# trustbloc/fabric-mod

Measured on AMD Instinct MI355X. Metric: ECDSA P-256 verifies/sec (whole node), higher is better.
Workload: dtype int64; 1 GPU; BASELINE.json configs[1]: block of 10000 tx x 3 endorsements = 30000 P-256 tuples per GPU, verify-only kernel via the C ABI, fresh keypair per signatu; tuples_per_gpu=30000, tx_per_block=10000, endorsements_per_tx=3, seed=20260921, parallelism=1 block per GPU, clock_warmup_launches=100

## Files before the change

fabric-mod_amd/csrc/fabgpu_api.hip:

```cpp
#include <hip/hip_runtime.h>
#include <stdlib.h>
#include <string.h>

#include <algorithm>
#include <atomic>
#include <chrono>
#include <condition_variable>
#include <initializer_list>
#include <memory>
#include <sys/mman.h>
#include <set>
#include <mutex>
#include <new>
#include <map>
#include <string>
#include <thread>
#include <vector>

#include "../../include/fabgpu.h"
#include "kernels.h"
#include "key_slots.h"
#include "keyed_fence.h"
#include "block_walk_dev.h"
#include "described_plan.h"
// ... 119 lines not shown
using HipKeyedFence = KeyedFence<HipFenceDev>;

}

struct fabgpu_ctx {
    int device = 0;
    bool allow_pair = true;
    bool allow_quad = true;
    bool nym_side_stream = true;
    std::atomic<bool> test_nym_side_after{false};
    bool nym_two_phase = true;
    bool allow_wide = true;
    int pair_table_lds = -1;
    bool pair_solo = false;
    bool pair_dbl1 = false;
    hipStream_t stream = nullptr;
    int fault = 0;
    int32_t* d_gtab = nullptr;
    uint32_t* d_gtab384 = nullptr;
    std::mutex gtab384_mu;
    std::mutex mu;
    Buf fields;
    Buf arena;
    Buf offs;
    Buf out;
    hipEvent_t ev0 = nullptr, ev1 = nullptr;
    bool timed = false;
    bool time_kernels = false;
    struct QWs {
        void* p = nullptr;
// ... 261 lines not shown
        default: return "unknown fabgpu error";
    }
}

int fabgpu_device_count(fabgpu_ctx*) {
    int n = 0;
    if (hipGetDeviceCount(&n) != hipSuccess) return FABGPU_ENODEV;
    return n;
}

int fabgpu_init(const fabgpu_cfg* cfg, fabgpu_ctx** out) {
    if (!out) return FABGPU_EINVAL;
    *out = nullptr;
    if (cfg && (cfg->flags & ~(uint32_t)(FABGPU_FLAG_ONE_LANE_ONLY | FABGPU_FLAG_TIME_KERNELS | FABGPU_FLAG_NO_QUAD | FABGPU_FLAG_PAIR_TABLE_LDS |
                                          FABGPU_FLAG_PAIR_TABLE_GLOBAL | FABGPU_FLAG_NO_WIDE | FABGPU_FLAG_NYM_FUSED_HASH | FABGPU_FLAG_NYM_NO_SIDE_STREAM |
                                          FABGPU_FLAG_KEY_TABLES_16BIT | FABGPU_FLAG_PAIR_SOLO | FABGPU_FLAG_PAIR_DBL1 | FABGPU_FLAG_P384_WIDE |
                                          FABGPU_FLAG_P384_KEY_TABLES_16BIT)) != 0) return FABGPU_EINVAL;
    if (cfg && (cfg->flags & FABGPU_FLAG_PAIR_TABLE_LDS) && (cfg->flags & FABGPU_FLAG_PAIR_TABLE_GLOBAL)) return FABGPU_EINVAL;
    int ndev = 0;
    if (hipGetDeviceCount(&ndev) != hipSuccess || ndev <= 0) return FABGPU_ENODEV;
    int dev = cfg ? cfg->device : -1;
    if (dev < 0) {
        if (hipGetDevice(&dev) != hipSuccess) return FABGPU_ENODEV;
    }
    if (dev >= ndev) return FABGPU_EINVAL;
    hipDeviceProp_t prop;
    if (hipGetDeviceProperties(&prop, dev) != hipSuccess) return FABGPU_ENODEV;
    if (strncmp(prop.gcnArchName, "gfx950", 6) != 0) return FABGPU_ENODEV;
    fabgpu_ctx* ctx = new (std::nothrow) fabgpu_ctx();
    if (!ctx) return FABGPU_ENOMEM;
    ctx->device = dev;
    ctx->walk_map.flags = hipHostMallocMapped | hipHostMallocCoherent;
    ctx->allow_pair = !(cfg && (cfg->flags & FABGPU_FLAG_ONE_LANE_ONLY));
    ctx->allow_quad = !(cfg && (cfg->flags & FABGPU_FLAG_NO_QUAD));
    ctx->nym_two_phase = !(cfg && (cfg->flags & FABGPU_FLAG_NYM_FUSED_HASH));
    ctx->nym_side_stream = !(cfg && (cfg->flags & FABGPU_FLAG_NYM_NO_SIDE_STREAM));
    ctx->key_tables_16 = cfg && (cfg->flags & FABGPU_FLAG_KEY_TABLES_16BIT);
    ctx->allow_wide = ctx->allow_pair && !(cfg && (cfg->flags & FABGPU_FLAG_NO_WIDE));
    ctx->pair_table_lds = cfg && (cfg->flags & FABGPU_FLAG_PAIR_TABLE_LDS) ? 1 : (cfg && (cfg->flags & FABGPU_FLAG_PAIR_TABLE_GLOBAL) ? 0 : pair_table_default());
    ctx->pair_solo = cfg && (cfg->flags & FABGPU_FLAG_PAIR_SOLO);
    ctx->pair_dbl1 = cfg && (cfg->flags & FABGPU_FLAG_PAIR_DBL1);
    if (std::max<size_t>(prop.sharedMemPerBlock, prop.maxSharedMemoryPerMultiProcessor) < (ctx->pair_solo ? pair_table_lds_solo_bytes() : pair_table_lds_bytes()))
        ctx->pair_table_lds = 0;
    ctx->time_kernels = cfg && (cfg->flags & FABGPU_FLAG_TIME_KERNELS);
    DeviceGuard g(dev);
    int rc = FABGPU_OK;
    do {
        if (hipStreamCreateWithFlags(&ctx->stream, hipStreamNonBlocking) != hipSuccess) { rc = FABGPU_ENODEV; break; }
        if (hipStreamCreateWithFlags(&ctx->stream2, hipStreamNonBlocking) != hipSuccess) { rc = FABGPU_ENODEV; break; }
        if (hipEventCreateWithFlags(&ctx->ev_up, hipEventDisableTiming) != hipSuccess) { rc = FABGPU_ENODEV; break; }
        if (hipStreamCreateWithFlags(&ctx->stream3, hipStreamNonBlocking) != hipSuccess) { rc = FABGPU_ENODEV; break; }
        if (hipStreamCreateWithFlags(&ctx->stream4, hipStreamNonBlocking) != hipSuccess) { rc = FABGPU_ENODEV; break; }
        if (hipStreamCreateWithFlags(&ctx->stream_copy, hipStreamNonBlocking) != hipSuccess) { rc = FABGPU_ENODEV; break; }
        {
            bool ok = true;
            for (auto& sc : ctx->stream_copy_more) ok = ok && hipStreamCreateWithFlags(&sc, hipStreamNonBlocking) == hipSuccess;
// ... 165 lines not shown
    if (hipEventElapsedTime(&ms, ctx->ev0, ctx->ev1) != hipSuccess) return -1.0f;
    return ms;
}
extern "C" {

int fabgpu_p256_verify_batch_dev(fabgpu_ctx* ctx, size_t n, const void* qx, const void* qy, const void* e, const void* r,
                                 const void* s, void* verdict_bits, void* status, void* stream) {
    if (!ctx || (n && (!qx || !qy || !e || !r || !s || !verdict_bits))) return FABGPU_EINVAL;
    if (dev_too_big(n)) return FABGPU_ETOOBIG;
    if (n == 0) return FABGPU_OK;
    DeviceGuard g(ctx->device);
    hipStream_t st = (hipStream_t)stream;
    VerifyLaunch v = verify_launch_common(ctx, n, r, s, verdict_bits, status);
    v.qx = qx; v.qy = qy;
    v.e = e;
    v.table_lds = ctx->pair_table_lds; v.pair_solo = ctx->pair_solo; v.pair_dbl1 = ctx->pair_dbl1;
    return timed_launch(ctx, st, verify_workspace_bytes((uint32_t)n, ctx->allow_pair), [&](void* wsp) {
        v.qws = wsp;
        return launch_verify(v, st);
    });
}

int fabgpu_sha256_batch_dev(fabgpu_ctx* ctx, size_t n, const void* arena, size_t arena_bytes, const void* off, void* digests,
                            void* stream) {
    if (!ctx || (n && (!arena || !off || !digests))) return FABGPU_EINVAL;
    if (dev_too_big(n, arena_bytes)) return FABGPU_ETOOBIG;
    if (n == 0) return FABGPU_OK;
    DeviceGuard g(ctx->device);
    hipStream_t st = (hipStream_t)stream;
    return timed_launch(ctx, st, 0, [&](void*) { return launch_sha256_batch((uint32_t)n, arena, arena_bytes, off, digests, st); });
}
// ... 2678 lines not shown
        v.n = tot.creators;
        v.e = dt + T.dig.off; v.r = a.r; v.s = a.s;
        v.gtab = ctx->d_gtab;
        v.verdict_bits = dt + T.bitc.off; v.status = dt + T.dst.off;
        v.allow_pair = true; v.lds_reserve = exclusive ? 84u << 10 : 0u;
        hipError_t e;
        if (keyed) {
            v.key_id = a.key_id; v.nkeys = nkeys; v.ktabs = (const void*)kt;
            e = launch_verify(v, s2);
        } else {
            size_t wi = 0;
            void* wsp = nullptr;
            int r2 = ctx->acquire_qws(verify_workspace_bytes(tot.creators, true), &wi, &wsp, s2);
            if (r2 != FABGPU_OK) return r2;
            v.qx = a.qx; v.qy = a.qy; v.qws = wsp;
            v.table_lds = ctx->pair_table_lds; v.pair_solo = ctx->pair_solo; v.pair_dbl1 = ctx->pair_dbl1;
            e = launch_verify(v, s2);
            ctx->release_qws(wi, s2);
        }
        return hip_to_rc(e);
    };
    auto finish = [&]() -> int {
        if (++ctx->walk_seq == 0) ++ctx->walk_seq;
        ho.seq = ctx->walk_seq;
        if (err == hipSuccess && nym_ran) err = hipStreamWaitEvent(st, ctx->ev_w[6], 0);
        if (err == hipSuccess && memo) err = hipMemsetAsync(dt + T.mslots.off, 0, T.mslots.bytes, st);
        if (err == hipSuccess && memo) err = hipMemsetAsync(&((WalkMemoTotals*)(dt + T.mtot.off))->live, 0, 4, st);
        mark("finish: memsets queued");
        if (!memo && !out.tuples && !out.tuple_digest && !out.tuple_qxy && !(has_nym_rows && out.nym_issuer) && walk_small_finish_fits(a, nc)) {
            if (err == hipSuccess) err = launch_walk_status_finish_small(a, nc, ho, st);
            mark("finish: last kernel queued");
// ... 399 lines not shown
```

fabric-mod_amd/csrc/kernels.h:

```cpp
#pragma once
#include <hip/hip_runtime_api.h>
#include <stddef.h>
#include <stdint.h>

namespace fab {
constexpr int KTAB_STRIDE = 4;
constexpr int KEY_SLOT_BITS = 12;
constexpr uint32_t KTAB_GEN_NONE = 0xFFFFFFFFu;
constexpr int VERIFY_BLOCK = 256;
constexpr int VERIFY_MAX_WGS = 256;
constexpr int VERIFY_PAIR_MAX = 32768;
constexpr size_t QWS_UINT4_PER_LANE = (size_t)16 * 8;
constexpr size_t QWS_PAIR_UINT4_PER_SIG = (size_t)16 * 8;

struct ShaPrefixArgs {
    uint32_t m = 0;
    const void* pre_off = nullptr;
    const void* pre_idx = nullptr;
    void* mid_scratch = nullptr;
    bool spans = false;
    void* digests = nullptr;
    bool mid_ready = false;
    uint32_t lds_reserve = 0;
};
// ... 19 lines not shown
    const void *qx = nullptr, *qy = nullptr;
    void* qws = nullptr;
    const void *key_id = nullptr, *ktabs = nullptr;
    uint32_t nkeys = 0;
    const void* e = nullptr;
    const void *arena = nullptr, *off = nullptr;
    size_t arena_bytes = 0;
    ShaPrefixArgs pa;
    const void *r = nullptr, *s = nullptr, *gtab = nullptr;
    void *verdict_bits = nullptr, *status = nullptr;
    bool allow_pair = false;
    uint32_t lds_reserve = 0;
    int table_lds = 0;
    bool pair_solo = false;
    bool pair_dbl1 = false;
};
hipError_t launch_verify(const VerifyLaunch& v, hipStream_t st);

constexpr int WIDE_LAUNCH_MAX = 8192;
constexpr size_t WIDE_SCRATCH_BYTES = 144;
constexpr uint32_t SPREAD_NONE = 0xFFFFFFFFu;
uint32_t spread_waves_per_cu(uint32_t wavefronts);
hipError_t launch_p256_wide_pre(uint32_t n, const void* key_id, uint32_t nkeys, const void* ktabs, const void* r, const void* s, const void* gtab,
                                void* scratch, hipStream_t st, uint32_t lds_spread = 0);
hipError_t launch_p256_wide_post(uint32_t n, const void* e, const void* r, const void* gtab, const void* scratch, void* verdict_bits, void* status,
                                 hipStream_t st, uint32_t lds_spread = 0);
hipError_t launch_sha256_messages(uint32_t n, const void* arena, size_t arena_bytes, const void* off, const ShaPrefixArgs& pa, hipStream_t st);
constexpr uint32_t SHA_COOP_MAX = 2048;
hipError_t launch_sha256_mixed(uint32_t n, const void* arena, size_t arena_bytes, const void* off, bool pairs, void* digests, hipStream_t st,
                               uint32_t lds_reserve = 0);
// ... 92 lines not shown
```

fabric-mod_amd/csrc/kernels.hip:

```cpp
#include <hip/hip_runtime.h>
#include <stdlib.h>
#include <stdint.h>

#include "device_common.h"
#include "kernels.h"
#include "p256_pair29.h"

namespace fab {


__global__ void __launch_bounds__(256) sha256_midstate_kernel(uint32_t m, const uint32_t* __restrict__ arena32, uint32_t arena_words,
                                                               const uint32_t* __restrict__ pre_off, uint32_t spans, uint32_t* __restrict__ mid) {
    uint32_t p = blockIdx.x * blockDim.x + threadIdx.x;
    bool active = p < m;
    uint32_t pc = active ? p : (m - 1);
    uint32_t start = pre_off[spans ? 2 * pc : pc], len = pre_off[spans ? 2 * pc + 1 : pc + 1] - start;
    uint32_t nfull = active ? (len >> 6) : 0, maxfull = nfull;
#pragma unroll
    for (int o = 32; o >= 1; o >>= 1) {
        uint32_t other = __shfl_xor(maxfull, o, 64);
        maxfull = other > maxfull ? other : maxfull;
    }
    maxfull = __builtin_amdgcn_readfirstlane(maxfull);
    uint32_t h[8];
// ... 60 lines not shown
struct DigestHashed {
    static constexpr bool BEFORE_KEY = true;
    const uint32_t* arena32;
    uint32_t arena_words;
    const uint32_t* off;
    const sha_prefixes pre;
    __device__ __forceinline__ void operator()(u256& ve, const TileRow& t, bool writes) const {
        uint32_t h[8];
        sha256_message(arena32, arena_words, off, pre, t.ic, t.active, h);
        emit_digest(pre, t.i, writes, h);
#pragma unroll
        for (int k = 0; k < 8; k++) ve.w[k] = h[7 - k];
    }
};

template <int LANE_COUNT, class QTab, int W = 5, bool DBL1 = false>
struct FreshKey {
    static constexpr int LANES = LANE_COUNT;
    const uint8_t *qx, *qy;
    const int32_t* gtab;
    QTab qtab;
    struct Row { u256 x, y; };
    __device__ __forceinline__ void load(Row& k, uint32_t ic) const {
        load_be_field(k.x, qx, ic);
        load_be_field(k.y, qy, ic);
    }
    __device__ __forceinline__ uint32_t verify(const Row& k, const u256& e, const u256& r, const u256& s, bool odd) {
        if constexpr (LANES == 1) {
            GTab16 gt{gtab};
            return p256_verify_core29(k.x, k.y, e, r, s, gt, qtab);
        } else {
            return p256_verify_pair29<QTab, W, DBL1>(k.x, k.y, e, r, s, gtab, qtab, odd);
        }
    }
};
template <int LANE_COUNT>
struct RegisteredKey {
    static constexpr int LANES = LANE_COUNT;
    const uint32_t* key_id;
    uint32_t nkeys;
    const int32_t* const* ktabs;
    const int32_t* gtab;
    struct Row { const int32_t *kt, *kt16; bool kok; };
    __device__ __forceinline__ void load(Row& k, uint32_t ic) const {
        const uint32_t kid = key_id[ic], sl = kid & ((1u << KEY_SLOT_BITS) - 1u);
        const bool inr = sl < nkeys;
        const int32_t* const* slot = ktabs + KTAB_STRIDE * (size_t)(inr ? sl : 0);
// ... 43 lines not shown
                                                                    uint8_t* __restrict__ status) {
    using QTab = GlobalQTab29<BLOCK>;
    verify_tiles<BLOCK>(n, DigestGiven{e}, FreshKey<1, QTab>{qx, qy, gtab, QTab::of(qws + (size_t)blockIdx.x * (QWS_UINT4_PER_LANE * BLOCK), threadIdx.x)}, r, s, verdict_bits, status);
}

template <int BLOCK>
__global__ void __launch_bounds__(BLOCK, 1) p256_verify_pair_kernel(uint32_t n, const uint8_t* __restrict__ qx, const uint8_t* __restrict__ qy,
                                                                         const uint8_t* __restrict__ e, const uint8_t* __restrict__ r,
                                                                         const uint8_t* __restrict__ s, const int32_t* __restrict__ gtab,
                                                                         uint4* __restrict__ qws, uint64_t* __restrict__ verdict_bits,
                                                                         uint8_t* __restrict__ status) {
    using QTab = PairQTab<BLOCK / 2>;
    verify_tiles<BLOCK>(n, DigestGiven{e}, FreshKey<2, QTab>{qx, qy, gtab, QTab::of(qws + (size_t)blockIdx.x * (QWS_PAIR_UINT4_PER_SIG * (BLOCK / 2)), threadIdx.x >> 1)}, r, s, verdict_bits, status);
}

template <int BLOCK, bool DBL1 = false>
__global__ void __launch_bounds__(BLOCK, 1) p256_verify_pair_lds_solo_kernel(uint32_t n, const uint8_t* __restrict__ qx, const uint8_t* __restrict__ qy,
                                                                             const uint8_t* __restrict__ e, const uint8_t* __restrict__ r,
                                                                             const uint8_t* __restrict__ s, const int32_t* __restrict__ gtab,
                                                                             uint64_t* __restrict__ verdict_bits, uint8_t* __restrict__ status) {
    extern __shared__ uint4 pair_lds[];
    verify_tiles<BLOCK>(n, DigestGiven{e}, FreshKey<2, PairQTabLds, 4, DBL1>{qx, qy, gtab, PairQTabLds::of(pair_lds, threadIdx.x >> 1)}, r, s, verdict_bits, status);
}

template <int BLOCK, bool DBL1 = false>
__global__ void __launch_bounds__(2 * BLOCK, 1) p256_verify_pair_lds_kernel(uint32_t n, const uint8_t* __restrict__ qx, const uint8_t* __restrict__ qy,
                                                                                 const uint8_t* __restrict__ e, const uint8_t* __restrict__ r,
                                                                                 const uint8_t* __restrict__ s, const int32_t* __restrict__ gtab,
                                                                                 uint64_t* __restrict__ verdict_bits, uint8_t* __restrict__ status) {
    extern __shared__ uint4 pair_lds[];
    using Geom = TileGeom<BLOCK, 2>;
    const bool helper = __builtin_amdgcn_readfirstlane(threadIdx.x) >= (uint32_t)BLOCK;
    const uint32_t lane = threadIdx.x & (uint32_t)(BLOCK - 1);
    const bool odd = Geom::odd(lane);
    const uint32_t sub = Geom::sub(lane);
    PairQTabLds qtab = PairQTabLds::of(pair_lds, sub);
    const PairHandoffLds<BLOCK> hand = PairHandoffLds<BLOCK>::of(reinterpret_cast<uint32_t*>(pair_lds + Geom::PER_WG * PAIR_LDS_CELLS_PER_SIG), lane);
    const uint32_t ntiles = Geom::ntiles(n);
    for (uint32_t tile = blockIdx.x; tile < ntiles; tile += gridDim.x) {
        const TileRow t = Geom::row(tile, sub, n);
        u256 u1;
        uint32_t early = 0;
        pair_pt Qp, T;
        bool q_ok = false, t_inf = true;
        if (helper) {
            u256 ve, vr, vs;
            load_be_field(ve, e, t.ic);
            load_be_field(vr, r, t.ic);
            load_be_field(vs, s, t.ic);
            pair_helper_scalars29(u1, early, ve, vr, vs, hand, odd);
        } else {
            u256 vqx, vqy;
            load_be_field(vqx, qx, t.ic);
            load_be_field(vqy, qy, t.ic);
            q_ok = pair_main_table29(Qp, vqx, vqy, qtab, odd);
        }
        __syncthreads();
        if (helper) {
            pair_helper_comb29(u1, early, gtab, hand, odd);
        } else {
            u256 u2;
            hand.get_u2(u2);
            pair_u2_mult29<PairQTabLds, 4, DBL1>(T, t_inf, u2, Qp, qtab, odd);
        }
        __syncthreads();
        if (!helper) {
            u256 vr;
            load_be_field(vr, r, t.ic);
            uint32_t st = pair_main_finish29(T, t_inf, q_ok, vr, hand, odd);
            Geom::emit(t, n, odd, st, verdict_bits, status);
        }
    }
}

template <int BLOCK>
__global__ void __launch_bounds__(BLOCK, 2) p256_verify_keyed_kernel(uint32_t n, const uint32_t* __restrict__ key_id, uint32_t nkeys,
                                                                          const int32_t* const* __restrict__ ktabs, const uint8_t* __restrict__ e,
                                                                          const uint8_t* __restrict__ r, const uint8_t* __restrict__ s,
// ... 127 lines not shown
    g.block = VERIFY_BLOCK;
    g.pair = allow_pair && n <= (uint32_t)VERIFY_PAIR_MAX;
    uint32_t per_wg = g.pair ? VERIFY_BLOCK / 2 : VERIFY_BLOCK;
    uint32_t tiles = (n + per_wg - 1) / per_wg;
    g.wgs = tiles < (uint32_t)VERIFY_MAX_WGS ? tiles : (uint32_t)VERIFY_MAX_WGS;
    return g;
}
int pair_table_default() { return -1; }
size_t pair_table_lds_bytes() { return (size_t)(VERIFY_BLOCK / 2) * PAIR_LDS_CELLS_PER_SIG * 16 + (size_t)VERIFY_BLOCK * PAIR_HAND_WORDS * 4; }
size_t pair_table_lds_solo_bytes() { return (size_t)(VERIFY_BLOCK / 2) * PAIR_LDS_CELLS_PER_SIG * 16; }
size_t verify_workspace_bytes(uint32_t n, bool allow_pair) {
    VerifyGeom g = verify_geom(n, allow_pair);
    if (g.pair) return (size_t)g.wgs * (g.block / 2) * QWS_PAIR_UINT4_PER_SIG * 16;
    return (size_t)g.wgs * g.block * QWS_UINT4_PER_LANE * 16;
}

hipError_t launch_verify(const VerifyLaunch& v, hipStream_t st) {
    const uint32_t n = v.n;
    if (n == 0) return hipSuccess;
    const bool keyed = v.key_id != nullptr && v.ktabs != nullptr, fresh = v.qx != nullptr && v.qy != nullptr;
    const bool hashed = v.off != nullptr, given = v.e != nullptr;
    if (keyed == fresh || hashed == given || keyed != (v.key_id != nullptr || v.ktabs != nullptr) || fresh != (v.qx != nullptr || v.qy != nullptr) ||
        (hashed && v.arena == nullptr && v.arena_bytes != 0))
        return hipErrorInvalidValue;
    const uint8_t *qx = (const uint8_t*)v.qx, *qy = (const uint8_t*)v.qy, *e = (const uint8_t*)v.e, *r = (const uint8_t*)v.r, *s = (const uint8_t*)v.s;
    const uint32_t *key_id = (const uint32_t*)v.key_id, *arena32 = (const uint32_t*)v.arena, *off = (const uint32_t*)v.off;
    const uint32_t arena_words = (uint32_t)((v.arena_bytes + 3) / 4);
    const int32_t* const* ktabs = (const int32_t* const*)v.ktabs;
    const int32_t* gtab = (const int32_t*)v.gtab;
    uint4* qws = (uint4*)v.qws;
    uint64_t* verdict_bits = (uint64_t*)v.verdict_bits;
    uint8_t* status = (uint8_t*)v.status;
    sha_prefixes pre{};
    if (hashed) pre = launch_midstates(v.arena, v.arena_bytes, v.pa, st);
    VerifyGeom g = verify_geom(n, v.allow_pair);
    dim3 grid(g.wgs), block(g.block);
    const uint32_t lds_reserve = hashed ? v.pa.lds_reserve : v.lds_reserve;
    if (!hashed && !keyed) {
        const bool table_lds = v.table_lds < 0 ? n > (uint32_t)PAIR_TABLE_LDS_FROM : v.table_lds != 0;
        if (g.pair && table_lds && !v.pair_solo && !v.pair_dbl1)
            hipLaunchKernelGGL(p256_verify_pair_lds_kernel<VERIFY_BLOCK>, grid, dim3(2 * VERIFY_BLOCK), pair_table_lds_bytes(), st, n, qx, qy, e, r, s, gtab, verdict_bits, status);
        else if (g.pair && table_lds && !v.pair_solo)
            hipLaunchKernelGGL((p256_verify_pair_lds_kernel<VERIFY_BLOCK, true>), grid, dim3(2 * VERIFY_BLOCK), pair_table_lds_bytes(), st, n, qx, qy, e, r, s, gtab, verdict_bits, status);
        else if (g.pair && table_lds && !v.pair_dbl1)
            hipLaunchKernelGGL(p256_verify_pair_lds_solo_kernel<VERIFY_BLOCK>, grid, block, pair_table_lds_solo_bytes(), st, n, qx, qy, e, r, s, gtab, verdict_bits, status);
        else if (g.pair && table_lds)
            hipLaunchKernelGGL((p256_verify_pair_lds_solo_kernel<VERIFY_BLOCK, true>), grid, block, pair_table_lds_solo_bytes(), st, n, qx, qy, e, r, s, gtab, verdict_bits, status);
        else if (g.pair)
            hipLaunchKernelGGL(p256_verify_pair_kernel<VERIFY_BLOCK>, grid, block, lds_reserve, st, n, qx, qy, e, r, s, gtab, qws, verdict_bits, status);
        else
            hipLaunchKernelGGL(p256_verify_kernel<VERIFY_BLOCK>, grid, block, lds_reserve, st, n, qx, qy, e, r, s, gtab, qws, verdict_bits, status);
        return hipGetLastError();
    }
    if (hashed && !keyed) {
        if (g.pair)
            hipLaunchKernelGGL(sha256_p256_verify_pair_kernel<VERIFY_BLOCK>, grid, block, lds_reserve, st, n, arena32, arena_words, off, qx, qy, r, s, gtab, qws,
                               verdict_bits, status, pre);
        else
            hipLaunchKernelGGL(sha256_p256_verify_kernel<VERIFY_BLOCK>, grid, block, lds_reserve, st, n, arena32, arena_words, off, qx, qy, r, s, gtab, qws,
                               verdict_bits, status, pre);
        return hipGetLastError();
    }
    if (!hashed) {
// ... 6 lines not shown
    if (g.pair)
        hipLaunchKernelGGL(sha256_p256_verify_keyed_pair_kernel<VERIFY_BLOCK>, grid, block, lds_reserve, st, n, arena32, arena_words, off, key_id, v.nkeys, ktabs,
                           r, s, gtab, verdict_bits, status, pre);
    else
        hipLaunchKernelGGL(sha256_p256_verify_keyed_kernel<VERIFY_BLOCK>, grid, block, lds_reserve, st, n, arena32, arena_words, off, key_id, v.nkeys, ktabs,
                           r, s, gtab, verdict_bits, status, pre);
    return hipGetLastError();
}

int warm_kernel_functions_kernels() {
    int ok = 0;
    hipFuncAttributes a;
    const void* fns[] = {(const void*)p256_verify_kernel<VERIFY_BLOCK>, (const void*)p256_verify_pair_kernel<VERIFY_BLOCK>,
                         (const void*)p256_verify_pair_lds_kernel<VERIFY_BLOCK>, (const void*)p256_verify_pair_lds_solo_kernel<VERIFY_BLOCK>,
                         (const void*)p256_verify_pair_lds_kernel<VERIFY_BLOCK, true>, (const void*)p256_verify_pair_lds_solo_kernel<VERIFY_BLOCK, true>,
                         (const void*)p256_verify_keyed_kernel<VERIFY_BLOCK>,
                         (const void*)p256_verify_keyed_pair_kernel<VERIFY_BLOCK>, (const void*)sha256_p256_verify_keyed_kernel<VERIFY_BLOCK>,
                         (const void*)sha256_p256_verify_keyed_pair_kernel<VERIFY_BLOCK>, (const void*)sha256_p256_verify_pair_kernel<VERIFY_BLOCK>,
                         (const void*)sha256_p256_verify_kernel<VERIFY_BLOCK>, (const void*)sha256_midstate_kernel, (const void*)gather_spans_kernel};
    for (const void* f : fns) ok += hipFuncGetAttributes(&a, f) == hipSuccess ? 1 : 0;
    return ok;
}

}
```

fabric-mod_amd/csrc/p256_pair29.h:

```cpp
#pragma once
#include "p256_verify29.h"
#include "pair29_gcn.h"

namespace fab {

struct pair_pt {
    fe A, B;
};

__device__ __forceinline__ int32_t pair_swap_i32(int32_t v) {
    return __builtin_amdgcn_update_dpp(0, v, 0xB1, 0xF, 0xF, false);
}
__device__ __forceinline__ void pair_swap_fe(fe& r, const fe& a) {
#pragma unroll
    for (int i = 0; i < 9; i++) r.v[i] = pair_swap_i32(a.v[i]);
}
__device__ __forceinline__ void pair_sel(pair_pt& r, bool c, const pair_pt& a, const pair_pt& b) {
    fe_sel(r.A, c, a.A, b.A);
    fe_sel(r.B, c, a.B, b.B);
}

#define PAIR_TMPS __attribute__((unused)) fe tU1, tU2, tU3, tU4, tU6, tW, tH, tRR, tP1, tP2, tT0, tT1, tTD
#define PAIR_DBL(P) PAIR29_DBL((P).A, (P).B, tU1, tU2, tU3, tW, tP1, tP2, tT0, tT1, tTD)
#define PAIR_DBL4(P) PAIR29_DBL4((P).A, (P).B, tU1, tU2, tU3, tP1, tT0, tTD, tW)
// ... 344 lines not shown
        bool special = true;
#pragma unroll
        for (int l = 0; l < 8; l++) special = special & (u2.w[l] == NM2.w[l]);
        if (__any(special)) {
            pair_pt two;
            qtab.load_state(2u, two, odd);
            fe ny;
#pragma unroll
            for (int l = 0; l < 9; l++) ny.v[l] = -two.B.v[l];
            fe_sel(two.B, odd, two.B, ny);
            pair_sel(T, special, two, T);
        }
    }
}

template <class QTab, int W = 5, bool DBL1 = false>
__device__ __forceinline__ void pair_combined_mult29(pair_pt& Rr, bool& r_inf, const u256& u1, const u256& u2, const fe& QX, const fe& QY,
                                                     const int32_t* __restrict__ gtab, const QTab& qtab, bool odd) {
    static_assert(W == 4 || W == 5, "signed 4- or 5-bit windows");
    const fe ONE = {FE29_R1};
    pair_pt Qp;
    Qp.A = QX;
    fe_sel(Qp.B, odd, ONE, QY);
    pair_qtab_build29<QTab, W>(Qp, QX, QY, qtab, odd);
    pair_pt T;
    bool t_inf;
    pair_u2_mult29<QTab, W, DBL1>(T, t_inf, u2, Qp, qtab, odd);

    pair_pt S;
    bool s_inf;
    pair_comb_mult29<GTab16>(S, s_inf, u1, gtab, Qp, odd);
    pair_final_add29(Rr, r_inf, S, s_inf, T, t_inf, odd);
}

template <class KTab = KeyTab8>
__device__ __forceinline__ void pair_combined_mult_keyed29(pair_pt& Rr, bool& r_inf, const u256& u1, const u256& u2,
                                                           const int32_t* __restrict__ gtab, const int32_t* __restrict__ ktab, bool odd) {
    const fe ONE = {FE29_R1};
    fe gx, gy;
    GTab16 gt{gtab};
    gt.load(0, 1u, gx, gy);
    pair_pt seed, S, T;
// ... 13 lines not shown
    fe_sqr(zz, Rr.B);
    fe_to_mont(rm, r);
    fe_mul(rhs, rm, zz);
    pair_swap_fe(rhs_e, rhs);
    fe_sub(d, rhs_e, Rr.A);
    bool ok = fe_is_zero(d);
    add256(r2, r, N);
    fe_to_mont(rm, r2);
    fe_mul(rhs, rm, zz);
    pair_swap_fe(rhs_e, rhs);
    fe_sub(d, rhs_e, Rr.A);
    ok = ok | (lt256(r, PMN) & fe_is_zero(d));
    return ok & !r_inf;
}

template <class QTab, int W = 5, bool DBL1 = false>
__device__ __forceinline__ uint32_t p256_verify_pair29(const u256& qx, const u256& qy, const u256& e, const u256& r, const u256& s,
                                                        const int32_t* __restrict__ gtab, const QTab& qtab, bool odd) {
    const u256 P = FAB_P256_P;
    uint32_t early = range_status(r, s);

    bool q_in_field = lt256(qx, P) & lt256(qy, P);
    fe QX, QY;
    fe_to_mont(QX, qx);
    fe_to_mont(QY, qy);
    bool q_ok = q_in_field & on_curve29(QX, QY);
    if (early == ST_VALID && !q_ok) early = ST_OFF_CURVE;

    u256 u1, u2;
    pair_ecdsa_scalars29(u1, u2, e, r, s, odd);

    pair_pt Rr;
    bool r_inf;
    pair_combined_mult29<QTab, W, DBL1>(Rr, r_inf, u1, u2, QX, QY, gtab, qtab, odd);
    bool ok = pair_x_equals_r29(Rr, r_inf, r);
    uint32_t st = ok ? ST_VALID : ST_BAD_MATH;
    return early != ST_VALID ? early : st;
}

__device__ __forceinline__ uint32_t p256_verify_keyed_pair29(const u256& e, const u256& r, const u256& s, const int32_t* __restrict__ gtab,
                                                              const int32_t* __restrict__ ktab, const int32_t* __restrict__ ktab16, bool odd) {
    uint32_t early = range_status(r, s);
    u256 u1, u2;
    pair_ecdsa_scalars29(u1, u2, e, r, s, odd);
    pair_pt Rr;
    bool r_inf;
    if (__all(ktab16 != nullptr)) pair_combined_mult_keyed29<GTab16>(Rr, r_inf, u1, u2, gtab, ktab16, odd);
    else pair_combined_mult_keyed29<KeyTab8>(Rr, r_inf, u1, u2, gtab, ktab, odd);
    bool ok = pair_x_equals_r29(Rr, r_inf, r);
// ... 26 lines not shown
#pragma unroll
        for (int l = 0; l < 9; l++) s[(9 + l) * LANES] = (uint32_t)S.B.v[l];
        s[18 * LANES] = (s_inf ? 1u : 0u) | (early << 1);
    }
    __device__ __forceinline__ void get_s(pair_pt& S, bool& s_inf, uint32_t& early) const {
#pragma unroll
        for (int l = 0; l < 9; l++) S.A.v[l] = (int32_t)s[l * LANES];
#pragma unroll
        for (int l = 0; l < 9; l++) S.B.v[l] = (int32_t)s[(9 + l) * LANES];
        uint32_t f = s[18 * LANES];
        s_inf = (f & 1u) != 0;
        early = f >> 1;
    }
};

template <class Hand>
__device__ __forceinline__ void pair_helper_scalars29(u256& u1, uint32_t& early, const u256& e, const u256& r, const u256& s, const Hand& hand,
                                                      bool odd) {
    early = range_status(r, s);
    u256 u2;
    pair_ecdsa_scalars29(u1, u2, e, r, s, odd);
    hand.put_u2(u2);
}

template <class Hand>
__device__ __forceinline__ void pair_helper_comb29(const u256& u1, uint32_t early, const int32_t* __restrict__ gtab, const Hand& hand, bool odd) {
    const fe ONE = {FE29_R1};
    fe gx, gy;
    GTab16 gt{gtab};
    gt.load(0, 1u, gx, gy);
    pair_pt seed, S;
    seed.A = gx;
    fe_sel(seed.B, odd, ONE, gy);
    bool s_inf;
    pair_comb_mult29<GTab16>(S, s_inf, u1, gtab, seed, odd);
    hand.put_s(S, s_inf, early);
}

template <class QTab>
__device__ __forceinline__ bool pair_main_table29(pair_pt& Qp, const u256& qx, const u256& qy, const QTab& qtab, bool odd) {
    const u256 P = FAB_P256_P;
    const fe ONE = {FE29_R1};
    bool q_in_field = lt256(qx, P) & lt256(qy, P);
    fe QX, QY;
    fe_to_mont(QX, qx);
    fe_to_mont(QY, qy);
    bool q_ok = q_in_field & on_curve29(QX, QY);
    Qp.A = QX;
    fe_sel(Qp.B, odd, ONE, QY);
    pair_qtab_build29<QTab, 4>(Qp, QX, QY, qtab, odd);
    return q_ok;
}

template <class Hand>
__device__ __forceinline__ uint32_t pair_main_finish29(const pair_pt& T, bool t_inf, bool q_ok, const u256& r, const Hand& hand, bool odd) {
    pair_pt S, Rr;
    bool s_inf, r_inf;
    uint32_t early;
    hand.get_s(S, s_inf, early);
    if (early == ST_VALID && !q_ok) early = ST_OFF_CURVE;
    pair_final_add29(Rr, r_inf, S, s_inf, T, t_inf, odd);
    bool ok = pair_x_equals_r29(Rr, r_inf, r);
    uint32_t st = ok ? ST_VALID : ST_BAD_MATH;
    return early != ST_VALID ? early : st;
}
// ... 3 lines not shown
```

fabric-mod_amd/fabgpu/__init__.py:

```python
from __future__ import annotations

import ctypes
import os
from typing import List, Optional, Sequence, Tuple

import numpy as np

_HERE = os.path.dirname(os.path.abspath(__file__))
_LIB_PATH = os.environ.get("FABGPU_LIB_PATH") or os.path.join(os.path.dirname(_HERE), "lib", "libfabgpu.so")

FABGPU_OK = 0
IDB_SPANS = 1
IDB_ARENA_STAGED = 2
IDB_SHA3_256 = 4
FABGPU_EINVAL = -1
FABGPU_EPOISONED = -6
FLAG_ONE_LANE_ONLY = 1
FLAG_TIME_KERNELS = 2
FLAG_NYM_NO_SIDE_STREAM = 128
FLAG_NYM_FUSED_HASH = 64
FLAG_NO_QUAD = 4
FLAG_PAIR_TABLE_LDS = 8
FLAG_PAIR_TABLE_GLOBAL = 16
FLAG_PAIR_SOLO = 1024
FLAG_PAIR_DBL1 = 2048
FLAG_KEY_TABLES_16BIT = 256
FLAG_NO_WIDE = 32
FLAG_P384_KEY_TABLES_16BIT = 8192
FLAG_P384_WIDE = 4096
ST_VALID, ST_BAD_MATH, ST_HIGH_S, ST_RANGE, ST_OFF_CURVE = 0, 1, 2, 3, 4

_u8p = ctypes.POINTER(ctypes.c_uint8)
_u32p = ctypes.POINTER(ctypes.c_uint32)
_u64p = ctypes.POINTER(ctypes.c_uint64)
_vp = ctypes.c_void_p
_sz = ctypes.c_size_t


class FabgpuError(RuntimeError):
    """Infrastructure failure (non-zero FABGPU_E*): the Go provider would fall back to bccsp/sw."""
# ... 1681 lines not shown
```

include/fabgpu.h:

```cpp
#ifndef FABGPU_H
#define FABGPU_H

#include <stddef.h>
#include <stdint.h>

#ifdef __cplusplus
extern "C" {
#endif

#define FABGPU_ABI_VERSION 6

#define FABGPU_OK 0
#define FABGPU_EINVAL (-1)
#define FABGPU_ENODEV (-2)
#define FABGPU_ENOMEM (-3)
#define FABGPU_ELAUNCH (-4)
#define FABGPU_ETOOBIG (-5)
#define FABGPU_EPOISONED (-6)

#define FABGPU_ST_VALID 0
#define FABGPU_ST_BAD_MATH 1
#define FABGPU_ST_HIGH_S 2
#define FABGPU_ST_RANGE 3
#define FABGPU_ST_OFF_CURVE 4

typedef struct fabgpu_ctx fabgpu_ctx;

#define FABGPU_FLAG_ONE_LANE_ONLY 1u
#define FABGPU_FLAG_NO_QUAD 4u
#define FABGPU_FLAG_TIME_KERNELS 2u
#define FABGPU_FLAG_PAIR_TABLE_LDS 8u
#define FABGPU_FLAG_PAIR_TABLE_GLOBAL 16u
#define FABGPU_FLAG_NO_WIDE 32u

#define FABGPU_FLAG_NYM_FUSED_HASH 64u
#define FABGPU_FLAG_NYM_NO_SIDE_STREAM 128u

#define FABGPU_FLAG_PAIR_SOLO 1024u
#define FABGPU_FLAG_PAIR_DBL1 2048u

#define FABGPU_FLAG_KEY_TABLES_16BIT 256u

#define FABGPU_FLAG_P384_WIDE 4096u

#define FABGPU_FLAG_P384_KEY_TABLES_16BIT 8192u
#define FABGPU_P384_MAX_TABLES16 32

typedef struct fabgpu_cfg {
    int32_t device;
    uint32_t max_batch;
    uint32_t max_arena;
    uint32_t flags;
} fabgpu_cfg;

// ... 205 lines not shown
```

Baseline: 56.89 million verifies/s.

## Use odd-only signed 4-bit window recoding for the u2·Q pair multiplication

Replaces the Booth-style signed 4-bit recoding of u2 with an odd-digit recoding. u2 is first folded to an odd scalar via n−u2 when it is even, so every window is a nonzero odd digit. The Q table then holds only odd multiples (1Q..15Q), built by repeated adds of 2Q. The main loop becomes branch-free with no point-at-infinity tracking, and a special fix-up covers the n−2 edge case. The old path stays available behind a new BOOTH4 flag, and kernel dispatch moves to a lookup table.

```diff
diff --git a/fabric-mod_amd/csrc/fabgpu_api.hip b/fabric-mod_amd/csrc/fabgpu_api.hip
--- a/fabric-mod_amd/csrc/fabgpu_api.hip
+++ b/fabric-mod_amd/csrc/fabgpu_api.hip
@@ -157,6 +157,7 @@
     int pair_table_lds = -1;
     bool pair_solo = false;
     bool pair_dbl1 = false;
+    bool pair_booth4 = false;
     hipStream_t stream = nullptr;
     int fault = 0;
     int32_t* d_gtab = nullptr;
@@ -448,7 +449,7 @@
     *out = nullptr;
     if (cfg && (cfg->flags & ~(uint32_t)(FABGPU_FLAG_ONE_LANE_ONLY | FABGPU_FLAG_TIME_KERNELS | FABGPU_FLAG_NO_QUAD | FABGPU_FLAG_PAIR_TABLE_LDS |
                                           FABGPU_FLAG_PAIR_TABLE_GLOBAL | FABGPU_FLAG_NO_WIDE | FABGPU_FLAG_NYM_FUSED_HASH | FABGPU_FLAG_NYM_NO_SIDE_STREAM |
-                                          FABGPU_FLAG_KEY_TABLES_16BIT | FABGPU_FLAG_PAIR_SOLO | FABGPU_FLAG_PAIR_DBL1 | FABGPU_FLAG_P384_WIDE |
+                                          FABGPU_FLAG_KEY_TABLES_16BIT | FABGPU_FLAG_PAIR_SOLO | FABGPU_FLAG_PAIR_DBL1 | FABGPU_FLAG_PAIR_BOOTH4 | FABGPU_FLAG_P384_WIDE |
                                           FABGPU_FLAG_P384_KEY_TABLES_16BIT)) != 0) return FABGPU_EINVAL;
     if (cfg && (cfg->flags & FABGPU_FLAG_PAIR_TABLE_LDS) && (cfg->flags & FABGPU_FLAG_PAIR_TABLE_GLOBAL)) return FABGPU_EINVAL;
     int ndev = 0;
@@ -474,6 +475,7 @@
     ctx->pair_table_lds = cfg && (cfg->flags & FABGPU_FLAG_PAIR_TABLE_LDS) ? 1 : (cfg && (cfg->flags & FABGPU_FLAG_PAIR_TABLE_GLOBAL) ? 0 : pair_table_default());
     ctx->pair_solo = cfg && (cfg->flags & FABGPU_FLAG_PAIR_SOLO);
     ctx->pair_dbl1 = cfg && (cfg->flags & FABGPU_FLAG_PAIR_DBL1);
+    ctx->pair_booth4 = cfg && (cfg->flags & FABGPU_FLAG_PAIR_BOOTH4);
     if (std::max<size_t>(prop.sharedMemPerBlock, prop.maxSharedMemoryPerMultiProcessor) < (ctx->pair_solo ? pair_table_lds_solo_bytes() : pair_table_lds_bytes()))
         ctx->pair_table_lds = 0;
     ctx->time_kernels = cfg && (cfg->flags & FABGPU_FLAG_TIME_KERNELS);
@@ -669,7 +671,7 @@
     VerifyLaunch v = verify_launch_common(ctx, n, r, s, verdict_bits, status);
     v.qx = qx; v.qy = qy;
     v.e = e;
-    v.table_lds = ctx->pair_table_lds; v.pair_solo = ctx->pair_solo; v.pair_dbl1 = ctx->pair_dbl1;
+    v.table_lds = ctx->pair_table_lds; v.pair_solo = ctx->pair_solo; v.pair_dbl1 = ctx->pair_dbl1; v.pair_booth4 = ctx->pair_booth4;
     return timed_launch(ctx, st, verify_workspace_bytes((uint32_t)n, ctx->allow_pair), [&](void* wsp) {
         v.qws = wsp;
         return launch_verify(v, st);
@@ -3378,7 +3380,7 @@
             int r2 = ctx->acquire_qws(verify_workspace_bytes(tot.creators, true), &wi, &wsp, s2);
             if (r2 != FABGPU_OK) return r2;
             v.qx = a.qx; v.qy = a.qy; v.qws = wsp;
-            v.table_lds = ctx->pair_table_lds; v.pair_solo = ctx->pair_solo; v.pair_dbl1 = ctx->pair_dbl1;
+            v.table_lds = ctx->pair_table_lds; v.pair_solo = ctx->pair_solo; v.pair_dbl1 = ctx->pair_dbl1; v.pair_booth4 = ctx->pair_booth4;
             e = launch_verify(v, s2);
             ctx->release_qws(wi, s2);
         }
diff --git a/fabric-mod_amd/csrc/hosttest_pair_odd.cpp b/fabric-mod_amd/csrc/hosttest_pair_odd.cpp
--- /dev/null
+++ b/fabric-mod_amd/csrc/hosttest_pair_odd.cpp
@@ -0,0 +1,80 @@
+#include <stdio.h>
+#include <stdlib.h>
+#include <string.h>
+
+#include "p256_odd4.h"
+
+using namespace fab;
+
+static bool parse(u256& r, const char* s) {
+    if (strlen(s) < 64) return false;
+    for (int w = 0; w < 8; w++) {
+        uint32_t v = 0;
+        for (int c = 0; c < 8; c++) {
+            const char ch = s[(7 - w) * 8 + c];
+            uint32_t d;
+            if (ch >= '0' && ch <= '9') d = (uint32_t)(ch - '0');
+            else if (ch >= 'a' && ch <= 'f') d = (uint32_t)(ch - 'a' + 10);
+            else if (ch >= 'A' && ch <= 'F') d = (uint32_t)(ch - 'A' + 10);
+            else return false;
+            v = (v << 4) | d;
+        }
+        r.w[w] = v;
+    }
+    return true;
+}
+
+static void answer(const u256& u2) {
+    u256 k;
+    u2_fold_odd(k, u2);
+    for (int w = 7; w >= 0; w--) printf("%08x", k.w[w]);
+    uint32_t kw[9];
+    for (int w = 0; w < 8; w++) kw[w] = k.w[w];
+    kw[8] = 0;
+    odd_digit walked[ODD4_WINDOWS];
+    odd_walk4 wk;
+    odd_walk4_start(wk, k);
+    for (int i = ODD4_WINDOWS - 1; i >= 0; i--) walked[i] = odd_walk4_next(wk);
+    for (int i = 0; i < ODD4_WINDOWS; i++) {
+        const odd_digit d = odd_digit4(kw, i);
+        if (d.entry != walked[i].entry || d.neg != walked[i].neg) {
+            printf(" walk differs at %d\n", i);
+            exit(3);
+        }
+        printf(" %c%u", d.neg ? '-' : '+', d.entry);
+    }
+    printf("\n");
+}
+
+int main(int argc, char** argv) {
+    FILE* in = stdin;
+    if (argc > 1 && strcmp(argv[1], "self") == 0) {
+        const char* own[] = {"0000000000000000000000000000000000000000000000000000000000000001",
+                             "0000000000000000000000000000000000000000000000000000000000000002",
+                             "ffffffff00000000ffffffffffffffffbce6faada7179e84f3b9cac2fc63254f",
+                             "ffffffff00000000ffffffffffffffffbce6faada7179e84f3b9cac2fc632550",
+                             "8000000000000000000000000000000000000000000000000000000000000000",
+                             "ffffffffffffffffffffffffffffffffffffffffffffffffffffffffffffffff"};
+        for (const char* s : own) {
+            u256 v;
+            if (!parse(v, s)) return 2;
+            answer(v);
+        }
+        return 0;
+    }
+    if (argc > 1 && !(in = fopen(argv[1], "r"))) {
+        fprintf(stderr, "cannot open %s\n", argv[1]);
+        return 2;
+    }
+    char line[256];
+    while (fgets(line, sizeof line, in)) {
+        u256 v;
+        if (!parse(v, line)) {
+            fprintf(stderr, "bad line: %s", line);
+            return 2;
+        }
+        answer(v);
+    }
+    if (in != stdin) fclose(in);
+    return 0;
+}
diff --git a/fabric-mod_amd/csrc/kernels.h b/fabric-mod_amd/csrc/kernels.h
--- a/fabric-mod_amd/csrc/kernels.h
+++ b/fabric-mod_amd/csrc/kernels.h
@@ -57,6 +57,7 @@
     int table_lds = 0;
     bool pair_solo = false;
     bool pair_dbl1 = false;
+    bool pair_booth4 = false;
 };
 hipError_t launch_verify(const VerifyLaunch& v, hipStream_t st);
 
diff --git a/fabric-mod_amd/csrc/kernels.hip b/fabric-mod_amd/csrc/kernels.hip
--- a/fabric-mod_amd/csrc/kernels.hip
+++ b/fabric-mod_amd/csrc/kernels.hip
@@ -98,7 +98,7 @@
     }
 };
 
-template <int LANE_COUNT, class QTab, int W = 5, bool DBL1 = false>
+template <int LANE_COUNT, class QTab, int W = 5, bool DBL1 = false, bool BOOTH4 = false>
 struct FreshKey {
     static constexpr int LANES = LANE_COUNT;
     const uint8_t *qx, *qy;
@@ -114,7 +114,7 @@
             GTab16 gt{gtab};
             return p256_verify_core29(k.x, k.y, e, r, s, gt, qtab);
         } else {
-            return p256_verify_pair29<QTab, W, DBL1>(k.x, k.y, e, r, s, gtab, qtab, odd);
+            return p256_verify_pair29<QTab, W, DBL1, BOOTH4>(k.x, k.y, e, r, s, gtab, qtab, odd);
         }
     }
 };
@@ -188,16 +188,16 @@
     verify_tiles<BLOCK>(n, DigestGiven{e}, FreshKey<2, QTab>{qx, qy, gtab, QTab::of(qws + (size_t)blockIdx.x * (QWS_PAIR_UINT4_PER_SIG * (BLOCK / 2)), threadIdx.x >> 1)}, r, s, verdict_bits, status);
 }
 
-template <int BLOCK, bool DBL1 = false>
+template <int BLOCK, bool DBL1 = false, bool BOOTH4 = false>
 __global__ void __launch_bounds__(BLOCK, 1) p256_verify_pair_lds_solo_kernel(uint32_t n, const uint8_t* __restrict__ qx, const uint8_t* __restrict__ qy,
                                                                              const uint8_t* __restrict__ e, const uint8_t* __restrict__ r,
                                                                              const uint8_t* __restrict__ s, const int32_t* __restrict__ gtab,
                                                                              uint64_t* __restrict__ verdict_bits, uint8_t* __restrict__ status) {
     extern __shared__ uint4 pair_lds[];
-    verify_tiles<BLOCK>(n, DigestGiven{e}, FreshKey<2, PairQTabLds, 4, DBL1>{qx, qy, gtab, PairQTabLds::of(pair_lds, threadIdx.x >> 1)}, r, s, verdict_bits, status);
-}
-
-template <int BLOCK, bool DBL1 = false>
+    verify_tiles<BLOCK>(n, DigestGiven{e}, FreshKey<2, PairQTabLds, 4, DBL1, BOOTH4>{qx, qy, gtab, PairQTabLds::of(pair_lds, threadIdx.x >> 1)}, r, s, verdict_bits, status);
+}
+
+template <int BLOCK, bool DBL1 = false, bool BOOTH4 = false>
 __global__ void __launch_bounds__(2 * BLOCK, 1) p256_verify_pair_lds_kernel(uint32_t n, const uint8_t* __restrict__ qx, const uint8_t* __restrict__ qy,
                                                                                  const uint8_t* __restrict__ e, const uint8_t* __restrict__ r,
                                                                                  const uint8_t* __restrict__ s, const int32_t* __restrict__ gtab,
@@ -222,12 +222,12 @@
             load_be_field(ve, e, t.ic);
             load_be_field(vr, r, t.ic);
             load_be_field(vs, s, t.ic);
-            pair_helper_scalars29(u1, early, ve, vr, vs, hand, odd);
+            pair_helper_scalars29<PairHandoffLds<BLOCK>, BOOTH4>(u1, early, ve, vr, vs, hand, odd);
         } else {
             u256 vqx, vqy;
             load_be_field(vqx, qx, t.ic);
             load_be_field(vqy, qy, t.ic);
-            q_ok = pair_main_table29(Qp, vqx, vqy, qtab, odd);
+            q_ok = pair_main_table29<PairQTabLds, BOOTH4>(Qp, vqx, vqy, qtab, odd);
         }
         __syncthreads();
         if (helper) {
@@ -235,7 +235,12 @@
         } else {
             u256 u2;
             hand.get_u2(u2);
-            pair_u2_mult29<PairQTabLds, 4, DBL1>(T, t_inf, u2, Qp, qtab, odd);
+            if constexpr (BOOTH4) {
+                pair_u2_mult29<PairQTabLds, 4, DBL1>(T, t_inf, u2, Qp, qtab, odd);
+            } else {
+                pair_u2_mult_odd29<PairQTabLds, DBL1>(T, u2, qtab, odd);
+                t_inf = false;
+            }
         }
         __syncthreads();
         if (!helper) {
@@ -393,6 +398,13 @@
     if (g.pair) return (size_t)g.wgs * (g.block / 2) * QWS_PAIR_UINT4_PER_SIG * 16;
     return (size_t)g.wgs * g.block * QWS_UINT4_PER_LANE * 16;
 }
+
+using PairLdsKernel = void (*)(uint32_t, const uint8_t*, const uint8_t*, const uint8_t*, const uint8_t*, const uint8_t*, const int32_t*, uint64_t*, uint8_t*);
+static const PairLdsKernel pair_lds_kernels[2][2][2] = {
+    {{p256_verify_pair_lds_kernel<VERIFY_BLOCK, false, false>, p256_verify_pair_lds_kernel<VERIFY_BLOCK, false, true>},
+     {p256_verify_pair_lds_kernel<VERIFY_BLOCK, true, false>, p256_verify_pair_lds_kernel<VERIFY_BLOCK, true, true>}},
+    {{p256_verify_pair_lds_solo_kernel<VERIFY_BLOCK, false, false>, p256_verify_pair_lds_solo_kernel<VERIFY_BLOCK, false, true>},
+     {p256_verify_pair_lds_solo_kernel<VERIFY_BLOCK, true, false>, p256_verify_pair_lds_solo_kernel<VERIFY_BLOCK, true, true>}}};
 
 hipError_t launch_verify(const VerifyLaunch& v, hipStream_t st) {
     const uint32_t n = v.n;
@@ -417,15 +429,11 @@
     const uint32_t lds_reserve = hashed ? v.pa.lds_reserve : v.lds_reserve;
     if (!hashed && !keyed) {
         const bool table_lds = v.table_lds < 0 ? n > (uint32_t)PAIR_TABLE_LDS_FROM : v.table_lds != 0;
-        if (g.pair && table_lds && !v.pair_solo && !v.pair_dbl1)
-            hipLaunchKernelGGL(p256_verify_pair_lds_kernel<VERIFY_BLOCK>, grid, dim3(2 * VERIFY_BLOCK), pair_table_lds_bytes(), st, n, qx, qy, e, r, s, gtab, verdict_bits, status);
-        else if (g.pair && table_lds && !v.pair_solo)
-            hipLaunchKernelGGL((p256_verify_pair_lds_kernel<VERIFY_BLOCK, true>), grid, dim3(2 * VERIFY_BLOCK), pair_table_lds_bytes(), st, n, qx, qy, e, r, s, gtab, verdict_bits, status);
-        else if (g.pair && table_lds && !v.pair_dbl1)
-            hipLaunchKernelGGL(p256_verify_pair_lds_solo_kernel<VERIFY_BLOCK>, grid, block, pair_table_lds_solo_bytes(), st, n, qx, qy, e, r, s, gtab, verdict_bits, status);
-        else if (g.pair && table_lds)
-            hipLaunchKernelGGL((p256_verify_pair_lds_solo_kernel<VERIFY_BLOCK, true>), grid, block, pair_table_lds_solo_bytes(), st, n, qx, qy, e, r, s, gtab, verdict_bits, status);
-        else if (g.pair)
+        if (g.pair && table_lds) {
+            const PairLdsKernel k = pair_lds_kernels[v.pair_solo ? 1 : 0][v.pair_dbl1 ? 1 : 0][v.pair_booth4 ? 1 : 0];
+            if (v.pair_solo) hipLaunchKernelGGL(k, grid, block, pair_table_lds_solo_bytes(), st, n, qx, qy, e, r, s, gtab, verdict_bits, status);
+            else hipLaunchKernelGGL(k, grid, dim3(2 * VERIFY_BLOCK), pair_table_lds_bytes(), st, n, qx, qy, e, r, s, gtab, verdict_bits, status);
+        } else if (g.pair)
             hipLaunchKernelGGL(p256_verify_pair_kernel<VERIFY_BLOCK>, grid, block, lds_reserve, st, n, qx, qy, e, r, s, gtab, qws, verdict_bits, status);
         else
             hipLaunchKernelGGL(p256_verify_kernel<VERIFY_BLOCK>, grid, block, lds_reserve, st, n, qx, qy, e, r, s, gtab, qws, verdict_bits, status);
@@ -462,6 +470,8 @@
     const void* fns[] = {(const void*)p256_verify_kernel<VERIFY_BLOCK>, (const void*)p256_verify_pair_kernel<VERIFY_BLOCK>,
                          (const void*)p256_verify_pair_lds_kernel<VERIFY_BLOCK>, (const void*)p256_verify_pair_lds_solo_kernel<VERIFY_BLOCK>,
                          (const void*)p256_verify_pair_lds_kernel<VERIFY_BLOCK, true>, (const void*)p256_verify_pair_lds_solo_kernel<VERIFY_BLOCK, true>,
+                         (const void*)p256_verify_pair_lds_kernel<VERIFY_BLOCK, false, true>, (const void*)p256_verify_pair_lds_solo_kernel<VERIFY_BLOCK, false, true>,
+                         (const void*)p256_verify_pair_lds_kernel<VERIFY_BLOCK, true, true>, (const void*)p256_verify_pair_lds_solo_kernel<VERIFY_BLOCK, true, true>,
                          (const void*)p256_verify_keyed_kernel<VERIFY_BLOCK>,
                          (const void*)p256_verify_keyed_pair_kernel<VERIFY_BLOCK>, (const void*)sha256_p256_verify_keyed_kernel<VERIFY_BLOCK>,
                          (const void*)sha256_p256_verify_keyed_pair_kernel<VERIFY_BLOCK>, (const void*)sha256_p256_verify_pair_kernel<VERIFY_BLOCK>,
diff --git a/fabric-mod_amd/csrc/p256_odd4.h b/fabric-mod_amd/csrc/p256_odd4.h
--- /dev/null
+++ b/fabric-mod_amd/csrc/p256_odd4.h
@@ -0,0 +1,55 @@
+#pragma once
+#include "fp256.h"
+
+namespace fab {
+
+constexpr int ODD4_WINDOWS = 64;
+
+FAB_HD void u2_fold_odd(u256& k, const u256& u2) {
+    const u256 N = FAB_P256_N;
+    u256 t;
+    sub256(t, N, u2);
+    const bool even = (u2.w[0] & 1u) == 0;
+    sel256(k, even, t, u2);
+    k.w[0] = (k.w[0] & ~1u) | (even ? 1u : 0u);
+}
+
+struct odd_digit {
+    uint32_t entry;
+    bool neg;
+};
+
+FAB_HD odd_digit odd_digit4_of(uint32_t h, bool top, bool sign) {
+    const bool upper = top | (h >= 8u);
+    odd_digit d;
+    d.entry = top ? (h & 7u) : (h >= 8u ? h - 8u : 7u - h);
+    d.neg = (!upper) != sign;
+    return d;
+}
+
+FAB_HD odd_digit odd_digit4(const uint32_t (&kw)[9], int i) {
+    const int p = 4 * i + 1;
+    const uint64_t two = ((uint64_t)kw[(p >> 5) + 1] << 32) | kw[p >> 5];
+    const uint32_t h = (uint32_t)(two >> (p & 31)) & 15u;
+    return odd_digit4_of(h, i == ODD4_WINDOWS - 1, (kw[0] & 1u) != 0);
+}
+
+struct odd_walk4 {
+    u256 h;
+    bool sign, top;
+};
+FAB_HD void odd_walk4_start(odd_walk4& w, const u256& k) {
+    for (int i = 0; i < 7; i++) w.h.w[i] = (k.w[i] >> 1) | (k.w[i + 1] << 31);
+    w.h.w[7] = k.w[7] >> 1;
+    w.sign = (k.w[0] & 1u) != 0;
+    w.top = true;
+}
+FAB_HD odd_digit odd_walk4_next(odd_walk4& w) {
+    const odd_digit d = odd_digit4_of(w.h.w[7] >> 28, w.top, w.sign);
+    for (int i = 7; i > 0; i--) w.h.w[i] = (w.h.w[i] << 4) | (w.h.w[i - 1] >> 28);
+    w.h.w[0] <<= 4;
+    w.top = false;
+    return d;
+}
+
+}
diff --git a/fabric-mod_amd/csrc/p256_pair29.h b/fabric-mod_amd/csrc/p256_pair29.h
--- a/fabric-mod_amd/csrc/p256_pair29.h
+++ b/fabric-mod_amd/csrc/p256_pair29.h
@@ -1,5 +1,6 @@
 #pragma once
 #include "p256_verify29.h"
+#include "p256_odd4.h"
 #include "pair29_gcn.h"
 
 namespace fab {
@@ -382,7 +383,78 @@
     }
 }
 
-template <class QTab, int W = 5, bool DBL1 = false>
+template <class QTab>
+__device__ __forceinline__ void pair_qtab_build_odd29(const pair_pt& Qp, const fe& QX, const fe& QY, const QTab& qtab, bool odd) {
+    PAIR_TMPS;
+    qtab.store_state(1, Qp, odd);
+    pair_pt d = Qp, cur;
+    PAIR_DBL(d);
+    qtab.store_state(PAIR_LDS_ENTRIES, d, odd);
+    PAIR_MADD(cur, d, QX, QY);
+    qtab.store_state(2, cur, odd);
+#pragma unroll 1
+    for (int j = 3; j <= PAIR_LDS_ENTRIES; j++) {
+        fe C, D;
+        qtab.load_crossed((uint32_t)PAIR_LDS_ENTRIES, C, D, odd);
+        pair_pt sum;
+        PAIR_ADD(sum, cur, C, D);
+        cur = sum;
+        qtab.store_state(j, cur, odd);
+    }
+}
+
+template <class QTab, bool DBL1 = false>
+__device__ __forceinline__ void pair_u2_mult_odd29(pair_pt& T, const u256& k, const QTab& qtab, bool odd) {
+    PAIR_TMPS;
+    odd_walk4 wk;
+    odd_walk4_start(wk, k);
+    {
+        const odd_digit top = odd_walk4_next(wk);
+        qtab.load_state(top.entry + 1u, T, odd);
+        fe ny;
+#pragma unroll
+        for (int l = 0; l < 9; l++) ny.v[l] = -T.B.v[l];
+        fe_sel(T.B, top.neg & !odd, ny, T.B);
+    }
+#pragma unroll 1
+    for (int i = ODD4_WINDOWS - 2; i >= 0; i--) {
+        const odd_digit dg = odd_walk4_next(wk);
+        fe C, D;
+        qtab.load_crossed(dg.entry + 1u, C, D, odd);
+        if constexpr (!DBL1) {
+            PAIR_DBL4(T);
+        } else {
+#pragma unroll 1
+            for (int j = 0; j < 4; j++) PAIR_DBL(T);
+        }
+        {
+            const int32_t nm = dg.neg ? -1 : 0, nc = dg.neg ? 1 : 0;
+#pragma unroll
+            for (int l = 0; l < 9; l++) D.v[l] = (D.v[l] ^ nm) + nc;
+        }
+        pair_pt sum;
+        PAIR_ADD(sum, T, C, D);
+        T = sum;
+    }
+    {
+        const u256 NM2 = {{0xFC63254Fu, 0xF3B9CAC2u, 0xA7179E84u, 0xBCE6FAADu, 0xFFFFFFFFu, 0xFFFFFFFFu, 0x00000000u, 0xFFFFFFFFu}};
+        bool special = (k.w[0] | 1u) == NM2.w[0];
+#pragma unroll
+        for (int l = 1; l < 8; l++) special = special & (k.w[l] == NM2.w[l]);
+        if (__any(special)) {
+            pair_pt two;
+            qtab.load_state(1u, two, odd);
+            PAIR_DBL(two);
+            fe ny;
+#pragma unroll
+            for (int l = 0; l < 9; l++) ny.v[l] = -two.B.v[l];
+            fe_sel(two.B, ((k.w[0] & 1u) == 0) & !odd, ny, two.B);
+            pair_sel(T, special, two, T);
+        }
+    }
+}
+
+template <class QTab, int W = 5, bool DBL1 = false, bool BOOTH4 = false>
 __device__ __forceinline__ void pair_combined_mult29(pair_pt& Rr, bool& r_inf, const u256& u1, const u256& u2, const fe& QX, const fe& QY,
                                                      const int32_t* __restrict__ gtab, const QTab& qtab, bool odd) {
     static_assert(W == 4 || W == 5, "signed 4- or 5-bit windows");
@@ -390,10 +462,18 @@
     pair_pt Qp;
     Qp.A = QX;
     fe_sel(Qp.B, odd, ONE, QY);
-    pair_qtab_build29<QTab, W>(Qp, QX, QY, qtab, odd);
     pair_pt T;
     bool t_inf;
-    pair_u2_mult29<QTab, W, DBL1>(T, t_inf, u2, Qp, qtab, odd);
+    if constexpr (W == 4 && !BOOTH4) {
+        pair_qtab_build_odd29<QTab>(Qp, QX, QY, qtab, odd);
+        u256 k;
+        u2_fold_odd(k, u2);
+        pair_u2_mult_odd29<QTab, DBL1>(T, k, qtab, odd);
+        t_inf = false;
+    } else {
+        pair_qtab_build29<QTab, W>(Qp, QX, QY, qtab, odd);
+        pair_u2_mult29<QTab, W, DBL1>(T, t_inf, u2, Qp, qtab, odd);
+    }
 
     pair_pt S;
     bool s_inf;
@@ -437,7 +517,7 @@
     return ok & !r_inf;
 }
 
-template <class QTab, int W = 5, bool DBL1 = false>
+template <class QTab, int W = 5, bool DBL1 = false, bool BOOTH4 = false>
 __device__ __forceinline__ uint32_t p256_verify_pair29(const u256& qx, const u256& qy, const u256& e, const u256& r, const u256& s,
                                                         const int32_t* __restrict__ gtab, const QTab& qtab, bool odd) {
     const u256 P = FAB_P256_P;
@@ -455,7 +535,7 @@
 
     pair_pt Rr;
     bool r_inf;
-    pair_combined_mult29<QTab, W, DBL1>(Rr, r_inf, u1, u2, QX, QY, gtab, qtab, odd);
+    pair_combined_mult29<QTab, W, DBL1, BOOTH4>(Rr, r_inf, u1, u2, QX, QY, gtab, qtab, odd);
     bool ok = pair_x_equals_r29(Rr, r_inf, r);
     uint32_t st = ok ? ST_VALID : ST_BAD_MATH;
     return early != ST_VALID ? early : st;
@@ -512,12 +592,17 @@
     }
 };
 
-template <class Hand>
+template <class Hand, bool BOOTH4 = false>
 __device__ __forceinline__ void pair_helper_scalars29(u256& u1, uint32_t& early, const u256& e, const u256& r, const u256& s, const Hand& hand,
                                                       bool odd) {
     early = range_status(r, s);
     u256 u2;
     pair_ecdsa_scalars29(u1, u2, e, r, s, odd);
+    if constexpr (!BOOTH4) {
+        u256 k;
+        u2_fold_odd(k, u2);
+        u2 = k;
+    }
     hand.put_u2(u2);
 }
 
@@ -535,7 +620,7 @@
     hand.put_s(S, s_inf, early);
 }
 
-template <class QTab>
+template <class QTab, bool BOOTH4 = false>
 __device__ __forceinline__ bool pair_main_table29(pair_pt& Qp, const u256& qx, const u256& qy, const QTab& qtab, bool odd) {
     const u256 P = FAB_P256_P;
     const fe ONE = {FE29_R1};
@@ -546,7 +631,8 @@
     bool q_ok = q_in_field & on_curve29(QX, QY);
     Qp.A = QX;
     fe_sel(Qp.B, odd, ONE, QY);
-    pair_qtab_build29<QTab, 4>(Qp, QX, QY, qtab, odd);
+    if constexpr (BOOTH4) pair_qtab_build29<QTab, 4>(Qp, QX, QY, qtab, odd);
+    else pair_qtab_build_odd29<QTab>(Qp, QX, QY, qtab, odd);
     return q_ok;
 }
 
diff --git a/fabric-mod_amd/fabgpu/__init__.py b/fabric-mod_amd/fabgpu/__init__.py
--- a/fabric-mod_amd/fabgpu/__init__.py
+++ b/fabric-mod_amd/fabgpu/__init__.py
@@ -24,6 +24,7 @@
 FLAG_PAIR_TABLE_GLOBAL = 16
 FLAG_PAIR_SOLO = 1024
 FLAG_PAIR_DBL1 = 2048
+FLAG_PAIR_BOOTH4 = 16384
 FLAG_KEY_TABLES_16BIT = 256
 FLAG_NO_WIDE = 32
 FLAG_P384_KEY_TABLES_16BIT = 8192
diff --git a/include/fabgpu.h b/include/fabgpu.h
--- a/include/fabgpu.h
+++ b/include/fabgpu.h
@@ -38,6 +38,7 @@
 
 #define FABGPU_FLAG_PAIR_SOLO 1024u
 #define FABGPU_FLAG_PAIR_DBL1 2048u
+#define FABGPU_FLAG_PAIR_BOOTH4 16384u
 
 #define FABGPU_FLAG_KEY_TABLES_16BIT 256u
 
```

Result: faster. 57.86 million verifies/s (median of 6 runs) (+1.7%).
